# lucasnewman/f5-tts-mlx

Hardware: AMD Instinct MI355X
Metric: mel_frames_per_sec (higher is better)
Workload: dtype f16 (IEEE-half MFMA operands, fp32 accumulate / residual stream / LayerNorm / softmax state; meets the 1e-3 gate); 1 GPU; BASELINE configs[1]: F5-TTS 335M, 32-point euler (=62 DiT forwards, CFG), batch 1/GPU x 10 s (N=937) utterances, hipGraph=True; f16 (IEEE half) MFMA operands IN PLACE OF BASELINE's bf16 -- same width and MFMA rate, three more significand bits; plain bf16 fails the 1e-3 parity gate, see sub.b1_bf16; global_batch=1, seq_len=937, parallelism=dp1 (utterance sharding)

## Files before the change

### f5_tts_mlx_amd/csrc/attention.hip

```cpp
#include "attention.hpp"

namespace F5_NS {

__device__ __forceinline__ bool attn_block_map(const F5AttnArgs& p, int qrows, int& bh, int& qblk) {
    if (gridDim.y != 1) {
        bh = blockIdx.y;
        qblk = blockIdx.x;
        return true;
    }
    const int nqb = (p.seq_len + qrows - 1) / qrows;
    const int s = blockIdx.x >> 3;
    qblk = s % nqb;
    bh = (s / nqb) * 8 + (blockIdx.x & 7);
    return bh < p.B * p.H;
}

template <bool SCALE>
__device__ __forceinline__ void attn_pin_args(const F5AttnArgs& p) {
    if (SCALE)
        asm volatile("" ::"s"(p.qk[0]), "s"(p.vt[0]), "s"(p.out[0]), "s"(p.kv_len), "s"(p.B), "s"(p.H), "s"(p.seq_len), "s"(p.npad), "s"(p.ldqk),
                     "s"(p.ldo), "s"(p.dmodel), "s"(p.scale), "s"(p.out8));
    else
        asm volatile("" ::"s"(p.qk[0]), "s"(p.vt[0]), "s"(p.out[0]), "s"(p.kv_len), "s"(p.B), "s"(p.H), "s"(p.seq_len), "s"(p.npad), "s"(p.ldqk),
                     "s"(p.ldo), "s"(p.dmodel), "s"(p.out8));
// ... 873 lines not shown
        krow[i] = attn_kperm(srow);
        kcol[i] = p.dmodel + h * 64 + schunk * 8;
        ldsoff[i] = (i * 256 + wave * 64) * 8;
#pragma unroll
        for (int pp = 0; pp < NP; ++pp) {
            kptr[pp][i] = p.qk[pp] + (rowbase + grp * 64 + krow[i]) * p.ldqk + kcol[i];
            vptr[pp][i] = p.vt[pp] + ((size_t)bh * 64 + srow) * p.npad + grp * 64 + schunk * 8;
        }
    }
    const size_t kstep = (size_t)64 * KS * p.ldqk;
#define A2S_ISSUE(jj_)                                                                                       \
    {                                                                                                        \
        op16_t* st_ = smem + ((jj_) % NST) * (NP * 2 * TILE);                                                \
        const int gt_ = (jj_) * KS + grp;                                                                    \
        const bool tail_ = (gt_ * 64 + 63) > p.seq_len - 1;                                                  \
        _Pragma("unroll") for (int i = 0; i < 2; ++i) {                                                      \
            _Pragma("unroll") for (int pp = 0; pp < NP; ++pp) {                                              \
                const op16_t* ks_ = kptr[pp][i];                                                             \
                if (tail_) {                                                                                 \
                    int key_ = gt_ * 64 + krow[i];                                                           \
                    if (key_ > p.seq_len - 1) key_ = p.seq_len - 1;                                          \
                    ks_ = p.qk[pp] + (rowbase + key_) * p.ldqk + kcol[i];                                    \
                }                                                                                            \
                attn_glds16(ks_, st_ + (pp * 2) * TILE + ldsoff[i]);                                         \
                attn_glds16(vptr[pp][i], st_ + (pp * 2 + 1) * TILE + ldsoff[i]);                             \
                kptr[pp][i] += kstep;                                                                        \
                vptr[pp][i] += 64 * KS;                                                                      \
            }                                                                                                \
        }                                                                                                    \
    }

    f32x16 o[2];
#pragma unroll
    for (int e = 0; e < 16; ++e) {
        o[0][e] = 0.0f;
        o[1][e] = 0.0f;
    }
    float m_run = -INFINITY, l_run = 0.0f;
    const float c2 = p.q_prescaled ? 1.0f : p.scale * 1.4426950408889634f;

    if (ntg > 0) A2S_ISSUE(0);
    if (NST == 3 && ntg > 1) A2S_ISSUE(1);
    ATTN_PIN_Q(qf, NP, 4);

    for (int jj = 0; jj < nit; ++jj) {
        attn_wait_barrier(NST == 3 && jj + 1 < ntg);
        if (jj + NST - 1 < ntg) A2S_ISSUE(jj + NST - 1);
        if (jj >= ntg) continue;

        const op16_t* st = smem + (jj % NST) * (NP * 2 * TILE);
        const op16_t* sK = st;
        const op16_t* sV = st + TILE;
        const op16_t* sKl = st + (NP - 1) * 2 * TILE;
        const op16_t* sVl = st + (NP - 1) * 2 * TILE + TILE;

        f32x16 s[2];
        const int key0 = (jj * KS + grp) * 64;
#define A2S_QK()                                                                                             \
        {                                                                                                    \
            __builtin_amdgcn_s_setprio(1);                                                                   \
            _Pragma("unroll") for (int kb = 0; kb < 2; ++kb) {                                               \
                _Pragma("unroll") for (int e = 0; e < 16; ++e) s[kb][e] = 0.0f;                              \
                _Pragma("unroll") for (int ks = 0; ks < 4; ++ks) {                                           \
                    const int off = attn_swz(kb * 32 + lq, ks * 2 + hi);                                     \
                    const op16x8 a = *reinterpret_cast<const op16x8*>(&sK[off]);                             \
                    s[kb] = F5_MFMA32(a, qf[0][ks], s[kb], 0, 0, 0);                                         \
                    if (HP) {                                                                                \
                        const op16x8 al = *reinterpret_cast<const op16x8*>(&sKl[off]);                       \
                        s[kb] = F5_MFMA32(al, qf[0][ks], s[kb], 0, 0, 0);                                    \
                        s[kb] = F5_MFMA32(a, qf[NP - 1][ks], s[kb], 0, 0, 0);                                \
                    }                                                                                        \
                }                                                                                            \
            }                                                                                                \
            __builtin_amdgcn_s_setprio(0);                                                                   \
            if (key0 + 64 > kvlen) {                                                                         \
                _Pragma("unroll") for (int kb = 0; kb < 2; ++kb)                                             \
                    _Pragma("unroll") for (int r = 0; r < 16; ++r) {                                         \
                        const int key = key0 + kb * 32 + 16 * hi + r;                                        \
                        if (key >= kvlen) s[kb][r] = -INFINITY;                                              \
                    }                                                                                        \
            }                                                                                                \
        }
        A2S_QK();
        float psum = 0.0f;
        bool slow = !FAST || HP || jj == 0;
        if (!slow) {
            const float mc = m_run * c2;
            attn_f32x2 ps2 = {0.0f, 0.0f};
            ps2 = attn_exp_block(s[0], c2, mc, ps2);
            ps2 = attn_exp_block(s[1], c2, mc, ps2);
            psum = ps2[0] + ps2[1];
            slow = __any(!(psum <= ATTN_SUM_LIMIT));
            if (slow) A2S_QK();
        }
        if (slow) {
            float tmax = -INFINITY;
#pragma unroll
            for (int kb = 0; kb < 2; ++kb)
#pragma unroll
                for (int r = 0; r < 16; ++r) tmax = fmaxf(tmax, s[kb][r]);
            tmax = fmaxf(tmax, __shfl_xor(tmax, 32, 64));
            if (__any(tmax > m_run)) {
                const float m_new = fmaxf(m_run, tmax);
                const float alpha = __builtin_amdgcn_exp2f((m_run - m_new) * c2);
                m_run = m_new;
                l_run *= alpha;
#pragma unroll
                for (int e = 0; e < 16; ++e) {
                    o[0][e] *= alpha;
                    o[1][e] *= alpha;
                }
            }
            const float mc = m_run * c2;
            attn_f32x2 ps2 = {0.0f, 0.0f};
            ps2 = attn_exp_block(s[0], c2, mc, ps2);
            ps2 = attn_exp_block(s[1], c2, mc, ps2);
            psum = ps2[0] + ps2[1];
        }
        l_run += psum;
#undef A2S_QK

#pragma unroll
        for (int ks4 = 0; ks4 < 4; ++ks4) {
            const int kb = ks4 >> 1, sp = ks4 & 1;
            uint32_t pw[4], pwl[4];
#pragma unroll
            for (int e = 0; e < 4; ++e) {
                const float p0 = s[kb][8 * sp + 2 * e], p1 = s[kb][8 * sp + 2 * e + 1];
                pw[e] = f5_pack2_bounded(p0, p1);
                if (HP) pwl[e] = f5_pack2_lo(p0, p1);
            }
            const op16x8 pb = __builtin_bit_cast(op16x8, u32x4{pw[0], pw[1], pw[2], pw[3]});
            op16x8 pbl = pb;
            if (HP) pbl = __builtin_bit_cast(op16x8, u32x4{pwl[0], pwl[1], pwl[2], pwl[3]});
            __builtin_amdgcn_s_setprio(1);
#pragma unroll
            for (int db = 0; db < 2; ++db) {
                const int voff = attn_swz(db * 32 + lq, 4 * kb + 2 * hi + sp);
                const op16x8 a = *reinterpret_cast<const op16x8*>(&sV[voff]);
                o[db] = F5_MFMA32(a, pb, o[db], 0, 0, 0);
                if (HP) {
                    const op16x8 al = *reinterpret_cast<const op16x8*>(&sVl[voff]);
                    o[db] = F5_MFMA32(al, pb, o[db], 0, 0, 0);
                    o[db] = F5_MFMA32(a, pbl, o[db], 0, 0, 0);
                }
            }
            __builtin_amdgcn_s_setprio(0);
        }
    }
#undef A2S_ISSUE

    __syncthreads();
    float* mrg = reinterpret_cast<float*>(smem_all);
    if (grp > 0) {
        float* dst = mrg + (size_t)((grp - 1) * 4 + wave) * 34 * 64 + lane;
        dst[0] = m_run;
        dst[64] = l_run;
#pragma unroll
        for (int db = 0; db < 2; ++db)
#pragma unroll
            for (int e = 0; e < 16; ++e) dst[(2 + db * 16 + e) * 64] = o[db][e];
    }
    __syncthreads();
    if (grp > 0) return;
    float m_all = m_run;
#pragma unroll
    for (int g = 1; g < KS; ++g) m_all = fmaxf(m_all, mrg[(size_t)((g - 1) * 4 + wave) * 34 * 64 + lane]);
    {
        const float a0 = __builtin_amdgcn_exp2f((m_run - m_all) * c2);
        l_run *= a0;
#pragma unroll
        for (int e = 0; e < 16; ++e) {
            o[0][e] *= a0;
            o[1][e] *= a0;
        }
    }
#pragma unroll
    for (int g = 1; g < KS; ++g) {
        const float* src = mrg + (size_t)((g - 1) * 4 + wave) * 34 * 64 + lane;
        const float ag = __builtin_amdgcn_exp2f((src[0] - m_all) * c2);
        l_run += src[64] * ag;
#pragma unroll
        for (int db = 0; db < 2; ++db)
#pragma unroll
            for (int e = 0; e < 16; ++e) o[db][e] += src[(2 + db * 16 + e) * 64] * ag;
    }

    const float l_tot = l_run + __shfl_xor(l_run, 32, 64);
    const float inv = 1.0f / l_tot;
    const int qr = q0 + lq;
    if (!HP && p.out8) {
        if (qr < p.seq_len) attn_store_f8(p, o, inv, rowbase + qr, h, hi);
    } else if (qr < p.seq_len) {
#pragma unroll
        for (int db = 0; db < 2; ++db)
#pragma unroll
            for (int rg = 0; rg < 4; ++rg) {
                const int d = db * 32 + 8 * rg + 4 * hi;
                const float v0 = o[db][rg * 4 + 0] * inv, v1 = o[db][rg * 4 + 1] * inv;
                const float v2 = o[db][rg * 4 + 2] * inv, v3 = o[db][rg * 4 + 3] * inv;
                const size_t off = (rowbase + qr) * p.ldo + h * 64 + d;
                *reinterpret_cast<u32x2*>(p.out[0] + off) = u32x2{f5_pack2_bounded(v0, v1), f5_pack2_bounded(v2, v3)};
                if (HP && p.out[1])
                    *reinterpret_cast<u32x2*>(p.out[1] + off) = u32x2{f5_pack2_lo(v0, v1), f5_pack2_lo(v2, v3)};
            }
    }
}

int f5_attn_wide = -1;
int f5_attn_kvsplit = -1;
int f5_attn_pipe = 0;

static dim3 attn_grid(const F5AttnArgs& a, int qrows) {
    const int nqb = f5_cdiv(a.seq_len, qrows);
    return dim3(nqb * 8 * f5_cdiv(a.B * a.H, 8), 1);
}

static F5AttnKernel attn_route(const F5AttnArgs& a) {
    int ks = f5_attn_kvsplit;
    if (ks < 0) {
        const long wgs = (long)f5_cdiv(a.seq_len, 128) * a.B * a.H;
        const int ntile = f5_cdiv(a.seq_len, 64);
        ks = (wgs <= 160 && ntile >= 8) ? 4 : ((wgs <= 320 && ntile >= 4) ? 2 : 1);
    }
    if (!a.hp && ks <= 1 &&
        (f5_attn_wide >= 1 || (f5_attn_wide < 0 && (long)f5_cdiv(a.seq_len, 256) * a.B * a.H >= 512))) {
        const bool pipe = (a.pipe < 0 ? f5_attn_pipe : a.pipe) && a.q_prescaled;
        return pipe ? F5A_V2P : (a.q_prescaled ? F5A_V2F_PRE : F5A_V2F);
    }
    if (ks > 1) return a.hp ? F5A_V2S_HP : (ks >= 4 ? F5A_V2S_KS4 : F5A_V2S_KS2);
    return a.hp ? F5A_V2_HP : F5A_V2;
}

static int attn_launch(const F5AttnArgs& a, hipStream_t stream, int& reached) {
    F5_REQUIRE(a.B > 0 && a.H > 0 && a.seq_len > 0, "attention: bad shape");
    F5_REQUIRE(a.npad % 64 == 0 && a.npad >= a.seq_len, "attention: npad must be a multiple of 64 and >= seq_len");
    F5_REQUIRE(a.ldqk % 8 == 0 && a.ldo % 4 == 0, "attention: bad leading dims");
    F5_REQUIRE(a.qk[0] && a.vt[0] && (a.out[0] || a.out8), "attention: null pointer");
    F5_REQUIRE(!a.out8 || (!a.hp && a.out8s && a.ldo8 % 4 == 0),
               "attention: fp8 output needs the bf16 ring kernels");
    F5_REQUIRE(!a.hp || (a.qk[1] && a.vt[1] && a.out[1]), "attention: bf16x3 needs lo buffers");
    const F5AttnKernel k = attn_route(a);
    const dim3 grid = attn_grid(a, 128), gw = attn_grid(a, 256);
    switch (k) {
        case F5A_V2_HP: hipLaunchKernelGGL(f5_attn2_kernel<true>, grid, dim3(256), 0, stream, a); break;
        case F5A_V2: hipLaunchKernelGGL(f5_attn2_kernel<false>, grid, dim3(256), 0, stream, a); break;
        case F5A_V2F_PRE: hipLaunchKernelGGL(f5_attn2f_kernel<true>, gw, dim3(256), 0, stream, a); break;
        case F5A_V2F: hipLaunchKernelGGL(f5_attn2f_kernel<false>, gw, dim3(256), 0, stream, a); break;
        case F5A_V2P: hipLaunchKernelGGL(f5_attn2p_kernel, gw, dim3(256), 0, stream, a); break;
        case F5A_V2S_HP: hipLaunchKernelGGL((f5_attn2s_kernel<true, 2, 2>), grid, dim3(512), 0, stream, a); break;
        case F5A_V2S_KS2: hipLaunchKernelGGL((f5_attn2s_kernel<false, 2, 3, true>), grid, dim3(512), 0, stream, a); break;
        case F5A_V2S_KS4: hipLaunchKernelGGL((f5_attn2s_kernel<false, 4, 2, true>), grid, dim3(1024), 0, stream, a); break;
        default: break;
    }
    F5_LAUNCH_CHECK();
    reached = k;
    return 0;
}

int f5_launch_attention(const F5AttnArgs& a, hipStream_t stream) {
    int reached = F5A_NONE;
    const int rc = attn_launch(a, stream, reached);
    f5dbg::last_attn_kernel = rc == 0 ? (reached | (a.out8 ? F5A_OUT8 : 0)) : F5A_NONE;
    return rc;
}
}
```

### f5_tts_mlx_amd/csrc/gemm.hip

```cpp
#include "gemm.hpp"
#include "gemm_dev.hpp"
#include "rowops.hpp"
#include "lnrow.hpp"

namespace F5_NS {



template <int MB, int NB>
struct ResidPre {
    float x[MB][16][NB];
    float bias[NB], gate[NB];
    uint32_t keep[MB][4];
};
template <int MB, int NB>
__device__ __forceinline__ void resid_preload(const F5GemmArgs& p, ResidPre<MB, NB>& q, int row0, int colbase, int lane) {
    const int hi = lane >> 5, lcol = lane & 31;
    const bool keep_words = p.rowkeep != nullptr && (reinterpret_cast<uintptr_t>(p.rowkeep) & 3) == 0;
#pragma unroll
    for (int nb = 0; nb < NB; ++nb) {
        const int c = colbase + nb * 32 + lcol;
        const bool ok = c < p.N;
        q.bias[nb] = (p.bias != nullptr && ok) ? p.bias[c] : 0.0f;
        q.gate[nb] = ok ? p.gate[c] : 0.0f;
// ... 198 lines not shown
        pa[ks] = &smem[0][0] + swz_off(wm * (32 * MB) + frow, ks * 2 + fk);
        pb[ks] = &smem[0][0] + BMt * BK + swz_off(wn * (32 * NB) + frow, ks * 2 + fk);
    }
    static_assert(2 * (BMt + BNt) * BK * 2 <= 65536, "both buffers must be addressable by ds_read immediates");
#define REG_STEP(CUR, tt_)                                                                                    \
    {                                                                                                         \
        if ((tt_) + 1 < T) LOAD_TILE();                                                                       \
        _Pragma("unroll") for (int ks = 0; ks < 4; ++ks) {                                                    \
            op16x8 af[MB], bfr[NB];                                                                           \
            _Pragma("unroll") for (int mb = 0; mb < MB; ++mb)                                                 \
                af[mb] = *reinterpret_cast<const op16x8*>(pa[ks] + (CUR) * (BMt + BNt) * BK + mb * 32 * BK);  \
            _Pragma("unroll") for (int nb = 0; nb < NB; ++nb)                                                 \
                bfr[nb] = *reinterpret_cast<const op16x8*>(pb[ks] + (CUR) * (BMt + BNt) * BK + nb * 32 * BK); \
            _Pragma("unroll") for (int mb = 0; mb < MB; ++mb)                                                 \
                _Pragma("unroll") for (int nb = 0; nb < NB; ++nb)                                             \
                    acc[mb][nb] = F5_MFMA32(af[mb], bfr[nb], acc[mb][nb], 0, 0, 0); \
        }                                                                                                     \
        if ((tt_) + 1 < T) STORE_TILE(1 - (CUR));                                                             \
        __syncthreads();                                                                                      \
    }
    for (int tt = 0; tt < T; tt += 2) {
        REG_STEP(0, tt);
        if (tt + 1 < T) REG_STEP(1, tt + 1);
    }
#undef REG_STEP
#undef LOAD_TILE
#undef STORE_TILE

    if (small_tile_staged<EPI, NB>() && n0 + BNt <= p.N && (p.debug_flags & 2) == 0) {
        static_assert(!small_tile_staged<EPI, NB>() || 4 * small_tile_stage_elems<NB>() <= 2 * (BMt + BNt) * BK, "staging fits");
        __syncthreads();
        staged_epilogue_bf16<EPI, MB, NB>(p, acc, &smem[0][0] + wave * small_tile_stage_elems<NB>(), m0 + wm * (32 * MB),
                                          n0 + wn * (32 * NB), lane);
        return;
    }
    gemm_epilogue<EPI, MB, NB>(p, acc, m0, n0, wm, wn, lane);
    if (EPI == EPI_RESID_GATE && p.ln_counter) resid_ln_tail(p, tm, BMt, (p.N + BNt - 1) / BNt);
}

int f5_gemm_order = 0;
static bool gemm_mfast(const F5GemmArgs& a) {
    if (f5_gemm_order == 1) return false;
    if (f5_gemm_order == 2) return true;
    const size_t a_bytes = (size_t)(a.a_row_mod > 0 ? a.a_row_mod : a.M) * a.K * 2 * (a.nseg == 3 ? 2 : 1);
    return a_bytes <= (size_t)4 << 20;
}
static int ring_order(const F5GemmArgs& a, int tiles_m, int tiles_n) {
    const bool band_ok = tiles_n % 4 == 0 && tiles_n >= 8 && (long)tiles_m * tiles_n <= 512 && tiles_m >= 8;
    if ((f5_gemm_order == 3 || f5_gemm_order == 0) && band_ok) return tiles_n | (4 << 20);
    if (f5_gemm_order == 3) return tiles_n;
    return gemm_mfast(a) ? -tiles_m : tiles_n;
}

template <int EPI, int MB, int NB, int NST, int WM = 2, int WN = 2, int KS = 1, int ABL = 0, int FOLD = 0>
__global__ __launch_bounds__(64 * WM * WN * KS) void f5_gemm_ring_kernel(F5GemmArgs p, int tiles_n, int ntiles) {
    constexpr int NTG = 64 * WM * WN;
    constexpr int BMt = 32 * MB * WM, BNt = 32 * NB * WN;
    constexpr int NA = BMt * 8 / NTG, NW = BNt * 8 / NTG;
    static_assert(NA * NTG == BMt * 8 && NW * NTG == BNt * 8, "tile rows must divide over the threads");
    constexpr int G = NA + NW;
    constexpr int STAGE = (BMt + BNt) * BK;
    constexpr int RING = NST * STAGE;
    static_assert(KS * RING * 2 <= 160 * 1024, "LDS budget");
    __shared__ __attribute__((aligned(16))) op16_t smem_all[KS * RING];

    asm volatile("" ::"s"(p.A[0]), "s"(p.W[0]), "s"(p.lda), "s"(p.ldw), "s"(p.K), "s"(p.nseg), "s"(p.M), "s"(p.N), "s"(p.a_row_mod),
                 "s"(p.debug_flags), "s"(tiles_n), "s"(ntiles));
    if (EPI == EPI_RESID_GATE)
        asm volatile("" ::"s"(p.bias), "s"(p.out_f32), "s"(p.ldo), "s"(p.gate), "s"(p.rowkeep), "s"(p.ln_counter));
    const int bid = blockIdx.x;
    const int q = ntiles >> 3, r = ntiles & 7;
    const int xcd = bid & 7, idx = bid >> 3;
    const int tile = (xcd < r ? xcd * (q + 1) : r * (q + 1) + (xcd - r) * q) + idx;
    int tm, tn;
    if (tiles_n >= (1 << 20)) {
        const int band = tiles_n >> 20, tnn = tiles_n & ((1 << 20) - 1);
        const int per_band = band * (ntiles / tnn);
        const int b = tile / per_band, rem = tile - b * per_band;
        tm = rem / band;
        tn = b * band + (rem - tm * band);
    } else if (tiles_n > 0) {
        tm = tile / tiles_n;
        tn = tile - tm * tiles_n;
    } else {
        tn = tile / (-tiles_n);
        tm = tile - tn * (-tiles_n);
    }
    const int m0 = tm * BMt, n0 = tn * BNt;

    const int tid = threadIdx.x;
    const int lane = tid & 63;
    const int wave_all = __builtin_amdgcn_readfirstlane(tid >> 6);
    const int grp = wave_all / (WM * WN), wave = wave_all % (WM * WN);
    const int tg = tid - grp * NTG;
    const int wm = wave / WN, wn = wave % WN;
    op16_t* smem = smem_all + grp * RING;

    uint32_t a_src[NA], w_src[NW];
    int a_dst[NA], w_dst[NW];
#pragma unroll
    for (int i = 0; i < NA; ++i) {
        const int q_ = i * NTG + tg;
        const int row = q_ >> 3, chunk = (q_ & 7) ^ ((row >> 1) & 7);
        int gr = m0 + row;
        if (gr > p.M - 1) gr = p.M - 1;
        if (p.a_row_mod > 0) gr = gr % p.a_row_mod;
        a_src[i] = ((uint32_t)gr * (uint32_t)p.lda + chunk * 8) * 2u;
        a_dst[i] = (i * NTG + wave * 64) * 8;
    }
#pragma unroll
    for (int i = 0; i < NW; ++i) {
        const int q_ = i * NTG + tg;
        const int row = q_ >> 3, chunk = (q_ & 7) ^ ((row >> 1) & 7);
        w_src[i] = ((uint32_t)(n0 + row) * (uint32_t)p.ldw + chunk * 8) * 2u;
        w_dst[i] = BMt * BK + (i * NTG + wave * 64) * 8;
    }
    const int kt = p.K / BK;
    const int T = kt * p.nseg;
    const int Tg = T > grp ? (T - grp + KS - 1) / KS : 0;
    const int nit = (T + KS - 1) / KS;
    int is_seg = 0, is_k0 = grp * BK;
    while (is_k0 >= p.K) {
        is_k0 -= p.K;
        ++is_seg;
    }
#define RING_ISSUE(ST_)                                                                                      \
    {                                                                                                        \
        op16_t* st_ = smem + (ST_) * STAGE;                                                                  \
        const char* Ap_ = reinterpret_cast<const char*>((is_seg == 1) ? p.A[1] : p.A[0]);                    \
        const char* Wp_ = reinterpret_cast<const char*>((is_seg == 2) ? p.W[1] : p.W[0]);                    \
        const uint32_t kb_ = (uint32_t)is_k0 * 2u;                                                           \
        _Pragma("unroll") for (int i = 0; i < NA; ++i)                                                       \
            glds16(reinterpret_cast<const op16_t*>(Ap_ + (a_src[i] + kb_)), st_ + a_dst[i]);                 \
        _Pragma("unroll") for (int i = 0; i < NW; ++i)                                                       \
            glds16(reinterpret_cast<const op16_t*>(Wp_ + (w_src[i] + kb_)), st_ + w_dst[i]);                 \
        is_k0 += KS * BK;                                                                                    \
        while (is_k0 >= p.K) {                                          \
            is_k0 -= p.K;                                                                                    \
            ++is_seg;                                                                                        \
        }                                                                                                    \
    }

    f32x16 acc[MB][NB];
#pragma unroll
    for (int i = 0; i < MB; ++i)
#pragma unroll
        for (int j = 0; j < NB; ++j)
#pragma unroll
            for (int e = 0; e < 16; ++e) acc[i][j][e] = 0.0f;

    constexpr bool PRE_RESID = EPI == EPI_RESID_GATE && MB * NB <= 3;
    ResidPre<PRE_RESID ? MB : 1, PRE_RESID ? NB : 1> rpre;
    const bool use_pre = PRE_RESID && p.ln_counter == nullptr && (p.debug_flags & (8 | 256)) == 0;
    if (PRE_RESID && use_pre && grp == 0 && FOLD != 1)
        resid_preload<PRE_RESID ? MB : 1, PRE_RESID ? NB : 1>(p, rpre, m0 + wm * (32 * MB), n0 + wn * (32 * NB), lane);
    static_assert(FOLD == 0 || (FOLD == 1 && PRE_RESID && NB == 2) || (FOLD == 2 && EPI == EPI_GELU_TANH && NB == 2 && KS == 1 && WM * WN == 8),
                  "fold producer = the preloaded residual epilogue on 64-column wave tiles; fold consumer = the 8-wave GELU launch");
    ResidStagedPre<FOLD == 1 ? NB : 1> spre_p;
    if constexpr (FOLD == 1) {
        if (grp == 0) resid_staged_preload<NB>(p, spre_p, m0 + wm * (32 * MB), n0 + wn * (32 * NB), lane);
    }
    FoldPre fpre_c;
    fold_prefetch_clear(fpre_c);
    FoldStatsPre<8> spre_c;
    fold_stats_clear(spre_c);
    if constexpr (FOLD == 2) fold_stats_request_tr<1>(p, spre_c, fpre_c, m0 + wm * 32, n0 + wn * 64, lane);

#pragma unroll
    for (int st = 0; st < NST - 1; ++st)
        if (st < Tg) RING_ISSUE(st);

    const int frow = lane & 31;
    const int fk = lane >> 5;
    constexpr int SPS = 65536 / (STAGE * 2) < NST ? 65536 / (STAGE * 2) : NST;
    static_assert(SPS >= 1, "a stage must fit the ds_read offset field");
    constexpr int NSET = (NST + SPS - 1) / SPS;
    const op16_t* pa[NSET][4];
    const op16_t* pb[NSET][4];
#pragma unroll
    for (int w2 = 0; w2 < NSET; ++w2)
#pragma unroll
        for (int ks = 0; ks < 4; ++ks) {
            pa[w2][ks] = smem + w2 * SPS * STAGE + swz_off(wm * (32 * MB) + frow, ks * 2 + fk);
            pb[w2][ks] = smem + w2 * SPS * STAGE + BMt * BK + swz_off(wn * (32 * NB) + frow, ks * 2 + fk);
        }
    op16x8 abl_frag;
#pragma unroll
    for (int e = 0; e < 8; ++e) abl_frag[e] = (op16_t)0;
    if (ABL & 4) asm volatile("" : "+v"(abl_frag));
#define RING_STEP(ST_, jj_, TR_)                                                                                       \
    {                                                                                                               \
         \
        if ((jj_) + NST - 2 < Tg) {                                                                                 \
            if (NST == 4) asm volatile("s_waitcnt vmcnt(%0)" ::"n"(2 * G) : "memory");                              \
            else if (NST == 3) asm volatile("s_waitcnt vmcnt(%0)" ::"n"(G) : "memory");                             \
            else asm volatile("s_waitcnt vmcnt(0)" ::: "memory");                                                   \
        } else {                                                                                                    \
            asm volatile("s_waitcnt vmcnt(0)" ::: "memory");                                                        \
        }                                                                                                           \
        asm volatile("" ::: "memory");                                                                              \
        if (!(ABL & 8)) __builtin_amdgcn_s_barrier();                                                               \
        asm volatile("" ::: "memory");                                                                              \
        if (!(ABL & 1) && (jj_) + NST - 1 < Tg) RING_ISSUE(((ST_) + NST - 1) % NST);  \
        if (!(KS > 1 && (jj_) >= Tg)) {               \
            constexpr int W2 = (ST_) / SPS, SL = (ST_) % SPS;                                                        \
            _Pragma("unroll") for (int ks = 0; ks < 4; ++ks) {                                                      \
                op16x8 af[MB], bfr[NB];                                                                             \
                _Pragma("unroll") for (int mb = 0; mb < MB; ++mb)                                                   \
                    af[mb] = (ABL & 4) ? abl_frag : *reinterpret_cast<const op16x8*>(pa[W2][ks] + SL * STAGE + mb * 32 * BK); \
                _Pragma("unroll") for (int nb = 0; nb < NB; ++nb)                                                   \
                    bfr[nb] = (ABL & 4) ? abl_frag : *reinterpret_cast<const op16x8*>(pb[W2][ks] + SL * STAGE + nb * 32 * BK); \
                _Pragma("unroll") for (int mb = 0; mb < MB; ++mb)                                                   \
                    _Pragma("unroll") for (int nb = 0; nb < NB; ++nb) {                                             \
                        if (ABL & 2) asm volatile("" ::"v"(af[mb]), "v"(bfr[nb]));                                  \
                        else if (TR_) acc[mb][nb] = F5_MFMA32(bfr[nb], af[mb], acc[mb][nb], 0, 0, 0);               \
                        else acc[mb][nb] = F5_MFMA32(af[mb], bfr[nb], acc[mb][nb], 0, 0, 0);                        \
                    }                                                                                               \
            }                                                                                                       \
        }                                                                                                           \
    }
    if constexpr (FOLD == 2) {
        if (NST == 4) asm volatile("s_waitcnt vmcnt(%0)" ::"n"(2 * G) : "memory");
        else asm volatile("s_waitcnt vmcnt(0)" ::: "memory");
        fold_stats_pin(spre_c);
        fold_stats_finish_tr<1>(p, spre_c, fpre_c, m0 + wm * 32, lane, p.fold_mean_out != nullptr && n0 == 0 && wn == 0);
        fold_prefetch_pin(fpre_c);
        for (int jj = 0; jj < nit; jj += NST) {
            RING_STEP(0, jj, true);
            if (NST > 1 && jj + 1 < nit) RING_STEP(1 % NST, jj + 1, true);
            if (NST > 2 && jj + 2 < nit) RING_STEP(2 % NST, jj + 2, true);
            if (NST > 3 && jj + 3 < nit) RING_STEP(3 % NST, jj + 3, true);
        }
        __syncthreads();
        static_assert(FOLD != 2 || WM * WN * (small_tile_stage_elems<NB>() * 2 + 512) <= RING * 2, "staging + c1 | c2 scratch fit in the ring");
        float* fl = reinterpret_cast<float*>(smem_all + WM * WN * small_tile_stage_elems<NB>()) + wave * 128;
        staged_epilogue_tr<EPI, MB, NB, true>(p, acc, smem_all + wave * small_tile_stage_elems<NB>(), m0 + wm * (32 * MB), n0 + wn * (32 * NB), lane,
                                              fl, &fpre_c);
        return;
    }
    constexpr bool QKV_TR_OK = EPI == EPI_QKV_ROPE && (32 * NB) % 64 == 0 && (NB & (NB - 1)) == 0 && KS == 1 && WM * WN == 8;
    if (QKV_TR_OK && p.rope_g4k != nullptr && n0 + wn * (32 * NB) < 2 * p.dmodel) {
        for (int jj = 0; jj < nit; jj += NST) {
            RING_STEP(0, jj, true);
            if (NST > 1 && jj + 1 < nit) RING_STEP(1 % NST, jj + 1, true);
            if (NST > 2 && jj + 2 < nit) RING_STEP(2 % NST, jj + 2, true);
            if (NST > 3 && jj + 3 < nit) RING_STEP(3 % NST, jj + 3, true);
        }
        __syncthreads();
        staged_epilogue_tr_rope<MB, NB>(p, acc, smem_all + wave * small_tile_stage_elems<NB>(), m0 + wm * (32 * MB), n0 + wn * (32 * NB),
                                        lane);
        return;
    }
    for (int jj = 0; jj < nit; jj += NST) {
        RING_STEP(0, jj, false);
        if (NST > 1 && jj + 1 < nit) RING_STEP(1 % NST, jj + 1, false);
        if (NST > 2 && jj + 2 < nit) RING_STEP(2 % NST, jj + 2, false);
        if (NST > 3 && jj + 3 < nit) RING_STEP(3 % NST, jj + 3, false);
    }
#undef RING_STEP
#undef RING_ISSUE
    constexpr int STG = small_tile_staged<EPI, NB>() ? WM * WN * small_tile_stage_elems<NB>() : 0;
    if (KS > 1) {
        constexpr int RED = MB * NB * 16 * 64;
        static_assert(KS == 1 || STG * 2 + (KS - 1) * WM * WN * RED * 4 <= KS * RING * 2, "reduction area fits in the rings");
        float* red = reinterpret_cast<float*>(smem_all + STG);
        __syncthreads();
        if (grp > 0) {
            float* dst = red + (size_t)((grp - 1) * (WM * WN) + wave) * RED + lane;
#pragma unroll
            for (int mb = 0; mb < MB; ++mb)
#pragma unroll
                for (int nb = 0; nb < NB; ++nb)
#pragma unroll
                    for (int e = 0; e < 16; ++e) dst[((mb * NB + nb) * 16 + e) * 64] = acc[mb][nb][e];
        }
        __syncthreads();
        if (grp > 0) {
            if (EPI == EPI_RESID_GATE && p.ln_counter) resid_ln_tail(p, tm, BMt, (p.N + BNt - 1) / BNt);
            return;
        }
#pragma unroll
        for (int g = 1; g < KS; ++g) {
            const float* src = red + (size_t)((g - 1) * (WM * WN) + wave) * RED + lane;
#pragma unroll
            for (int mb = 0; mb < MB; ++mb)
#pragma unroll
                for (int nb = 0; nb < NB; ++nb)
#pragma unroll
                    for (int e = 0; e < 16; ++e) acc[mb][nb][e] += src[((mb * NB + nb) * 16 + e) * 64];
        }
    }
    if (small_tile_staged<EPI, NB>() && n0 + BNt <= p.N && (p.debug_flags & 2) == 0) {
        static_assert(STG <= RING, "staging fits");
        if (KS == 1) __syncthreads();
        staged_epilogue_bf16<EPI, MB, NB>(p, acc, smem_all + wave * small_tile_stage_elems<NB>(), m0 + wm * (32 * MB),
                                          n0 + wn * (32 * NB), lane);
        return;
    }
    if constexpr (FOLD == 1) {
        constexpr int RED_BYTES = (KS - 1) * WM * WN * MB * NB * 16 * 64 * 4;
        static_assert(RED_BYTES + WM * WN * 32 * (32 * NB + 4) * 4 <= KS * RING * 2, "staging behind the reduction area");
        float* stg = reinterpret_cast<float*>(reinterpret_cast<char*>(smem_all) + RED_BYTES) + wave * (32 * (32 * NB + 4));
        staged_epilogue_resid<MB, NB, true>(p, acc, stg, m0 + wm * (32 * MB), n0 + wn * (32 * NB), lane, &spre_p);
        return;
    }
    if constexpr (PRE_RESID) {
        if (use_pre) {
            resid_epilogue_preloaded<MB, NB>(p, acc, rpre, m0 + wm * (32 * MB), n0 + wn * (32 * NB), lane);
            return;
        }
    }
    gemm_epilogue<EPI, MB, NB>(p, acc, m0, n0, wm, wn, lane);
    if (EPI == EPI_RESID_GATE && p.ln_counter) resid_ln_tail(p, tm, BMt, (p.N + BNt - 1) / BNt);
}

template <int EPI, int MB, int NB, int NST, int WM = 2, int WN = 2, int KS = 1, int FOLD = 0>
static int launch_ring(const F5GemmArgs& a, hipStream_t stream) {
    const int tiles_m = f5_cdiv(a.M, 32 * MB * WM), tiles_n = f5_cdiv(a.N, 32 * NB * WN);
    const int ntiles = tiles_m * tiles_n;
    const int order = ring_order(a, tiles_m, tiles_n);
    hipLaunchKernelGGL((f5_gemm_ring_kernel<EPI, MB, NB, NST, WM, WN, KS, 0, FOLD>), dim3(ntiles), dim3(64 * WM * WN * KS), 0, stream, a, order, ntiles);
    F5_LAUNCH_CHECK();
    return 0;
}

template <int EPI, int MB, int NB>
static int launch_cfg(const F5GemmArgs& a, hipStream_t stream) {
    const int tiles_m = f5_cdiv(a.M, 64 * MB), tiles_n = f5_cdiv(a.N, 64 * NB);
    const int ntiles = tiles_m * tiles_n;
    hipLaunchKernelGGL((f5_gemm_kernel<EPI, MB, NB>), dim3(ntiles), dim3(256), 0, stream, a, tiles_n, ntiles);
    F5_LAUNCH_CHECK();
    return 0;
}

int f5_gemm_debug_flags = 0;

constexpr int FC_ROWS = 4, FC_MAXC = 8;
int f5_fold_consts_mfma = 1;
__global__ __launch_bounds__(256) void f5_fold_consts_kernel(const op16_t* __restrict__ w, int ldw, const float* __restrict__ bias,
                                                             const float* __restrict__ scale, const float* __restrict__ shift, size_t vec_stride,
                                                             int nvec, float* __restrict__ c1, float* __restrict__ c2, size_t out_stride, int N,
                                                             int K, F5FoldBatch bt) {
    w += (size_t)blockIdx.y * bt.w_stride;
    if (bias) bias += (size_t)blockIdx.y * bt.bias_stride;
    scale += (size_t)blockIdx.y * bt.mod_stride;
    shift += (size_t)blockIdx.y * bt.mod_stride;
    c1 += (size_t)blockIdx.y * bt.out_blk_stride;
    c2 += (size_t)blockIdx.y * bt.out_blk_stride;
    const int lane = threadIdx.x & 63, wave = threadIdx.x >> 6;
    const int n0 = (blockIdx.x * 4 + wave) * FC_ROWS;
    if (n0 >= N) return;
    const int nchunk = K >> 8;
    float wv[FC_ROWS][FC_MAXC][4];
#pragma unroll
    for (int r = 0; r < FC_ROWS; ++r) {
        const int n = n0 + r < N ? n0 + r : N - 1;
#pragma unroll
        for (int c = 0; c < FC_MAXC; ++c) {
            if (c < nchunk) {
                const op16x4 t = *reinterpret_cast<const op16x4*>(w + (size_t)n * ldw + c * 256 + lane * 4);
#pragma unroll
                for (int e = 0; e < 4; ++e) wv[r][c][e] = f5_op2f(t[e]);
            } else {
#pragma unroll
                for (int e = 0; e < 4; ++e) wv[r][c][e] = 0.0f;
            }
        }
    }
    for (int v = 0; v < nvec; ++v) {
        const float* sv = scale + (size_t)v * vec_stride;
        const float* bv = shift + (size_t)v * vec_stride;
        float a1[FC_ROWS], a2[FC_ROWS];
#pragma unroll
        for (int r = 0; r < FC_ROWS; ++r) a1[r] = a2[r] = 0.0f;
#pragma unroll
        for (int c = 0; c < FC_MAXC; ++c) {
            if (c < nchunk) {
                const f32x4 s4 = *reinterpret_cast<const f32x4*>(sv + c * 256 + lane * 4);
                const f32x4 b4 = *reinterpret_cast<const f32x4*>(bv + c * 256 + lane * 4);
#pragma unroll
                for (int r = 0; r < FC_ROWS; ++r)
#pragma unroll
                    for (int e = 0; e < 4; ++e) {
                        a1[r] += wv[r][c][e] * (1.0f + s4[e]);
                        a2[r] += wv[r][c][e] * b4[e];
                    }
            }
        }
#pragma unroll
        for (int r = 0; r < FC_ROWS; ++r) {
            a1[r] = f5_wave_sum(a1[r]);
            a2[r] = f5_wave_sum(a2[r]);
        }
        if (lane == 0) {
#pragma unroll
            for (int r = 0; r < FC_ROWS; ++r)
                if (n0 + r < N) {
                    c1[(size_t)v * out_stride + n0 + r] = a1[r];
                    c2[(size_t)v * out_stride + n0 + r] = a2[r] + (bias ? bias[n0 + r] : 0.0f);
                }
        }
    }
}

template <int NVB>
__global__ __launch_bounds__(256) void f5_fold_consts_mfma_kernel(const op16_t* __restrict__ w, int ldw, const float* __restrict__ bias,
                                                                  const float* __restrict__ scale, const float* __restrict__ shift,
                                                                  size_t vec_stride, int nvec, float* __restrict__ c1, float* __restrict__ c2,
                                                                  size_t out_stride, int N, int K, F5FoldBatch bt) {
    w += (size_t)blockIdx.y * bt.w_stride;
    if (bias) bias += (size_t)blockIdx.y * bt.bias_stride;
    scale += (size_t)blockIdx.y * bt.mod_stride;
    shift += (size_t)blockIdx.y * bt.mod_stride;
// ... 241 lines not shown
```

Before: 13560 mel-frames/s.

## Distribute split-K and split-KV reduction epilogues across all wave groups

In the split-K GEMM and the split-KV attention merge, the partial-result reduction and epilogue now run on every wave group, each owning a slice of the output columns, instead of being done only by group 0 after the others park their partials. Each group writes the slices it does not own to shared memory, then sums or softmax-merges its own slice and runs the epilogue on it, including residual preloading and staged output stores. The intent is to remove the serial tail where most waves sit idle while one group does all the reduction and stores. In exchange it adds shared-memory traffic and extra code paths with tighter LDS capacity assertions.

```diff
diff --git a/f5_tts_mlx_amd/csrc/attention.hip b/f5_tts_mlx_amd/csrc/attention.hip
--- a/f5_tts_mlx_amd/csrc/attention.hip
+++ b/f5_tts_mlx_amd/csrc/attention.hip
@@ -1049,6 +1049,95 @@
 
     __syncthreads();
     float* mrg = reinterpret_cast<float*>(smem_all);
+    if (HP || !p.out8) {
+        constexpr int Q = 32 / KS, NPK = 2 + 32 - Q;
+        constexpr int SLD = 64 + 8;
+        static_assert(KS * 4 * NPK * 64 * 4 + (HP ? 0 : 128 * SLD * 2) <= KS * RING * 2, "merge area + output staging fit in the rings");
+        float* mine = mrg + (size_t)((grp * 4 + wave) * NPK) * 64 + lane;
+        mine[0] = m_run;
+        mine[64] = l_run;
+#pragma unroll
+        for (int g = 0; g < KS; ++g)
+            if (grp == g) {
+#pragma unroll
+                for (int i = 0; i < 32; ++i)
+                    if (i / Q != g) mine[(2 + (i < g * Q ? i : i - Q)) * 64] = o[i >> 4][i & 15];
+            }
+        __syncthreads();
+        const float* src[KS];
+        float mg[KS];
+#pragma unroll
+        for (int g = 0; g < KS; ++g) {
+            src[g] = mrg + (size_t)((g * 4 + wave) * NPK) * 64 + lane;
+            mg[g] = src[g][0];
+        }
+        float m_all = mg[0];
+#pragma unroll
+        for (int g = 1; g < KS; ++g) m_all = fmaxf(m_all, mg[g]);
+        float ag[KS];
+#pragma unroll
+        for (int g = 0; g < KS; ++g) ag[g] = __builtin_amdgcn_exp2f((mg[g] - m_all) * c2);
+        float l_all = __builtin_fmaf(src[0][64], ag[0], src[1][64] * ag[1]);
+#pragma unroll
+        for (int g = 2; g < KS; ++g) l_all = __builtin_fmaf(src[g][64], ag[g], l_all);
+        float own[Q];
+#pragma unroll
+        for (int g = 0; g < KS; ++g)
+            if (grp == g) {
+#pragma unroll
+                for (int j = 0; j < Q; ++j) {
+                    const int i = g * Q + j;
+                    float w[KS];
+#pragma unroll
+                    for (int k = 0; k < KS; ++k) {
+                        w[k] = ag[k];
+                        asm volatile("" : "+v"(w[k]));
+                    }
+                    float x[KS];
+#pragma unroll
+                    for (int k = 0; k < KS; ++k) x[k] = k == g ? o[i >> 4][i & 15] : src[k][(2 + (i < k * Q ? i : i - Q)) * 64];
+                    float acc;
+                    if (KS == 2) {
+                        acc = __builtin_fmaf(x[0], w[0], x[1] * w[1]);
+                    } else {
+                        acc = x[0] * w[0];
+#pragma unroll
+                        for (int k = 1; k < KS; ++k) acc = __builtin_fmaf(x[k], w[k], acc);
+                    }
+                    own[j] = acc;
+                }
+            }
+        const float l_tot = l_all + __shfl_xor(l_all, 32, 64);
+        const float inv = 1.0f / l_tot;
+        const int qr = q0 + lq;
+        op16_t* stg = reinterpret_cast<op16_t*>(mrg + KS * 4 * NPK * 64);
+#pragma unroll
+        for (int j = 0; j < Q; j += 4) {
+            const int i = grp * Q + j;
+            const int d = (i >> 4) * 32 + 8 * ((i & 15) >> 2) + 4 * hi;
+            const float v0 = own[j] * inv, v1 = own[j + 1] * inv, v2 = own[j + 2] * inv, v3 = own[j + 3] * inv;
+            const u32x2 pk = {f5_pack2_bounded(v0, v1), f5_pack2_bounded(v2, v3)};
+            if (HP) {
+                if (qr < p.seq_len) {
+                    const size_t off = (rowbase + qr) * p.ldo + h * 64 + d;
+                    *reinterpret_cast<u32x2*>(p.out[0] + off) = pk;
+                    if (p.out[1]) *reinterpret_cast<u32x2*>(p.out[1] + off) = u32x2{f5_pack2_lo(v0, v1), f5_pack2_lo(v2, v3)};
+                }
+            } else {
+                *reinterpret_cast<u32x2*>(&stg[(wave * 32 + lq) * SLD + d]) = pk;
+            }
+        }
+        if (HP) return;
+        __syncthreads();
+#pragma unroll
+        for (int c = tid; c < 128 * 8; c += 256 * KS) {
+            const int row = c >> 3, ch = c & 7;
+            const int qrow = qblk * 128 + row;
+            if (qrow < p.seq_len)
+                *reinterpret_cast<u32x4*>(p.out[0] + (rowbase + qrow) * p.ldo + h * 64 + ch * 8) = *reinterpret_cast<const u32x4*>(&stg[row * SLD + ch * 8]);
+        }
+        return;
+    }
     if (grp > 0) {
         float* dst = mrg + (size_t)((grp - 1) * 4 + wave) * 34 * 64 + lane;
         dst[0] = m_run;
diff --git a/f5_tts_mlx_amd/csrc/gemm.hip b/f5_tts_mlx_amd/csrc/gemm.hip
--- a/f5_tts_mlx_amd/csrc/gemm.hip
+++ b/f5_tts_mlx_amd/csrc/gemm.hip
@@ -374,7 +374,14 @@
     constexpr bool PRE_RESID = EPI == EPI_RESID_GATE && MB * NB <= 3;
     ResidPre<PRE_RESID ? MB : 1, PRE_RESID ? NB : 1> rpre;
     const bool use_pre = PRE_RESID && p.ln_counter == nullptr && (p.debug_flags & (8 | 256)) == 0;
-    if (PRE_RESID && use_pre && grp == 0 && FOLD != 1)
+    constexpr bool SHARE = KS > 1 && NB == KS && FOLD == 0 && EPI != EPI_QKV_ROPE;
+    const bool share = SHARE && p.ln_counter == nullptr && (p.debug_flags & (8 | 256)) == 0;
+    constexpr bool SHARE_PRE = SHARE && PRE_RESID;
+    ResidPre<SHARE_PRE ? MB : 1, 1> rown;
+    if constexpr (SHARE_PRE) {
+        if (use_pre) resid_preload<MB, 1>(p, rown, m0 + wm * (32 * MB), n0 + wn * (32 * NB) + grp * 32, lane);
+    }
+    if (PRE_RESID && !SHARE_PRE && use_pre && grp == 0 && FOLD != 1)
         resid_preload<PRE_RESID ? MB : 1, PRE_RESID ? NB : 1>(p, rpre, m0 + wm * (32 * MB), n0 + wn * (32 * NB), lane);
     static_assert(FOLD == 0 || (FOLD == 1 && PRE_RESID && NB == 2) || (FOLD == 2 && EPI == EPI_GELU_TANH && NB == 2 && KS == 1 && WM * WN == 8),
                   "fold producer = the preloaded residual epilogue on 64-column wave tiles; fold consumer = the 8-wave GELU launch");
@@ -481,6 +488,59 @@
     }
 #undef RING_STEP
 #undef RING_ISSUE
+    if constexpr (SHARE) {
+        if (share) {
+            constexpr int RED1 = MB * 16 * 64;
+            constexpr int STG1 = small_tile_staged<EPI, 1>() ? small_tile_stage_elems<1>() : 0;
+            constexpr int STGS = KS * WM * WN * STG1;
+            static_assert(STGS * 2 + WM * WN * NB * (KS - 1) * RED1 * 4 <= KS * RING * 2, "staging + parked parts fit in the rings");
+            float* red = reinterpret_cast<float*>(smem_all + STGS) + (size_t)wave * (NB * (KS - 1) * RED1) + lane;
+            __syncthreads();
+#pragma unroll
+            for (int g = 0; g < KS; ++g)
+                if (grp == g) {
+#pragma unroll
+                    for (int nb = 0; nb < NB; ++nb)
+                        if (nb != g) {
+                            float* dst = red + (nb * (KS - 1) + (g < nb ? g : g - 1)) * RED1;
+#pragma unroll
+                            for (int mb = 0; mb < MB; ++mb)
+#pragma unroll
+                                for (int e = 0; e < 16; ++e) dst[(mb * 16 + e) * 64] = acc[mb][nb][e];
+                        }
+                }
+            __syncthreads();
+            f32x16 own[MB][1];
+#pragma unroll
+            for (int g = 0; g < KS; ++g)
+                if (grp == g) {
+                    const float* src = red + g * (KS - 1) * RED1;
+#pragma unroll
+                    for (int mb = 0; mb < MB; ++mb)
+#pragma unroll
+                        for (int e = 0; e < 16; ++e) {
+                            const float mine = acc[mb][g][e];
+                            float s = g == 0 ? mine : src[(mb * 16 + e) * 64];
+#pragma unroll
+                            for (int h = 1; h < KS; ++h) s += h == g ? mine : src[(h < g ? h : h - 1) * RED1 + (mb * 16 + e) * 64];
+                            own[mb][0][e] = s;
+                        }
+                }
+            const int row0 = m0 + wm * (32 * MB), col0 = n0 + wn * (32 * NB) + grp * 32;
+            if (small_tile_staged<EPI, NB>() && n0 + BNt <= p.N && (p.debug_flags & 2) == 0) {
+                staged_epilogue_bf16<EPI, MB, 1>(p, own, smem_all + wave_all * STG1, row0, col0, lane);
+                return;
+            }
+            if constexpr (SHARE_PRE) {
+                if (use_pre) {
+                    resid_epilogue_preloaded<MB, 1>(p, own, rown, row0, col0, lane);
+                    return;
+                }
+            }
+            gemm_epilogue<EPI, MB, 1>(p, own, m0, col0, wm, 0, lane);
+            return;
+        }
+    }
     constexpr int STG = small_tile_staged<EPI, NB>() ? WM * WN * small_tile_stage_elems<NB>() : 0;
     if (KS > 1) {
         constexpr int RED = MB * NB * 16 * 64;
```

New measurement: 13750 mel-frames/s, median of 6. 1.01x the previous value.
